# pierluigiferrari/fcn8s_tensorflow

Hardware: AMD Instinct MI355X
Metric: training images/sec at 1024x512 bs16 (higher is better)
Workload: dtype f32; 1 GPU; FCN-8s (VGG-16, fc6 7x7, 20 classes) train step, 1024x512, 16 images/GPU, SGD+momentum, keep_prob 0.5; global_batch=16, parallelism=dp1

## Files before the change

fcn8s_tensorflow_amd/csrc/elementwise.hip:

```cpp
#include "fcn8s_internal.h"
#include "cv_resize.h"
#include <math.h>
#include <map>
#include <mutex>
#include <stdio.h>
#include <stdlib.h>

namespace fcn8s {

static inline int cap_blocks(long long work, int per_block)
{
    long long b = (work + per_block - 1) / per_block;
    if (b > 2048) b = 2048;
    if (b < 1) b = 1;
    return (int)b;
}

__global__ void preprocess_kernel(const void* img, int dtype, float4* out, long long npix)
{
    const float m0 = 103.939f, m1 = 116.779f, m2 = 123.68f;
    for (long long p = blockIdx.x * (long long)blockDim.x + threadIdx.x; p < npix;
         p += (long long)gridDim.x * blockDim.x) {
        float r, g, b;
        if (dtype == 0) {
// ... 419 lines not shown
            const float4* src = reinterpret_cast<const float4*>(logits) + p0 * U;
#pragma unroll
            for (int i = 0; i < U; ++i) { const int u = i * 64 + lane; if (p0 * U + u < nunits) wp[u] = src[u]; }
            __builtin_amdgcn_wave_barrier();
#pragma unroll
            for (int i = 0; i < U; ++i) { const float4 t = wp[lane * U + i]; v[4*i] = t.x; v[4*i+1] = t.y; v[4*i+2] = t.z; v[4*i+3] = t.w; }
            __builtin_amdgcn_wave_barrier();
        } else {
            const float4 t = p < npix ? reinterpret_cast<const float4*>(logits)[p] : make_float4(0.f, 0.f, 0.f, 0.f);
            v[0] = t.x; v[1] = t.y; v[2] = t.z; v[3] = t.w;
        }
        float4 g[U];
#pragma unroll
        for (int i = 0; i < U; ++i) g[i] = make_float4(0.f, 0.f, 0.f, 0.f);
        if (pix >= 0) {
            float m = v[0];
#pragma unroll
            for (int i = 1; i < C; ++i) m = fmaxf(m, v[i]);
            float e[C]; float s = 0.f;
#pragma unroll
            for (int i = 0; i < C; ++i) { e[i] = expf(v[i] - m); s += e[i]; }
            const int lab = labels[pix];
            const bool ign = lab >= C;
            float vl = 0.f;
#pragma unroll
            for (int i = 0; i < C; ++i) vl = (i == lab) ? v[i] : vl;
            float gs = gscale;
            bool keep = !ign;
            if constexpr (PH == XENT_PLAIN) {
                if (!ign) lsum += (double)(m + logf(s) - vl);
            } else if constexpr (PH == XENT_WEIGHTED) {
                float w = ign ? 0.f : wsh[lab];
                if constexpr (PX) w *= tab[x.codes[pix]];
                gs = gscale * w; nv += !ign;
                if (!ign) lsum += (double)w * (double)(m + logf(s) - vl);
            } else if constexpr (PH == XENT_OHEM_LOSS) {
                const float l = m + logf(s) - vl;
                if (!ign) { ++nv; ntau += l >= x.tau; atomicAdd(&hsh[__float_as_uint(l) >> 21], 1u); }
                x.lbuf[pix] = ign ? -1.f : l;
            } else {
                const float l = x.lbuf[pix];
                keep = !ign && l >= tsel;
                float w = keep ? wsh[lab] : 0.f;
                if constexpr (PX) w *= tab[x.codes[pix]];
                gs = gsel * w;
                if (keep) lsum += (double)w * (double)l;
            }
            if (PH != XENT_OHEM_LOSS && dlogits) {
                const float inv = keep ? gs / s : 0.f;
#pragma unroll
                for (int i = 0; i < U; ++i) {
                    float4 t;
                    t.x = e[4*i] * inv - ((4*i) == lab ? gs : 0.f);
                    t.y = e[4*i+1] * inv - ((4*i+1) == lab ? gs : 0.f);
                    t.z = e[4*i+2] * inv - ((4*i+2) == lab ? gs : 0.f);
                    t.w = e[4*i+3] * inv - ((4*i+3) == lab ? gs : 0.f);
                    g[i] = t;
                    csum[4*i] += t.x; csum[4*i+1] += t.y; csum[4*i+2] += t.z; csum[4*i+3] += t.w;
                }
            }
        }
        if (PH != XENT_OHEM_LOSS && dlogits) {
            if constexpr (U > 1) {
#pragma unroll
                for (int i = 0; i < U; ++i) wp[lane * U + i] = g[i];
                __builtin_amdgcn_wave_barrier();
                float4* dst = reinterpret_cast<float4*>(dlogits) + p0 * U;
#pragma unroll
                for (int i = 0; i < U; ++i) { const int u = i * 64 + lane; if (p0 * U + u < nunits) dst[u] = wp[u]; }
                __builtin_amdgcn_wave_barrier();
            } else if (p < npix) reinterpret_cast<float4*>(dlogits)[p] = g[0];
        }
    }
    if constexpr (PH == XENT_WEIGHTED || PH == XENT_OHEM_LOSS) xent_fold<PH>(nv, ntau, cnt, hsh, x);
// ... 697 lines not shown
```

fcn8s_tensorflow_amd/csrc/fcn8s_internal.h:

```cpp
#pragma once
#include <hip/hip_runtime.h>
#include <stdint.h>
#include <cmath>
#include "../../include/fcn8s_hip.h"

#if defined(__HIP_DEVICE_COMPILE__) && !defined(__gfx950__)
#error "libfcn8s_hip is written for gfx950 (MI355X) only: build with --offload-arch=gfx950"
#endif
#define FCN8S_LDS_BYTES_NEEDED (160u * 1024u)

#include <string>
namespace fcn8s {

extern thread_local const char* g_last_kernel;
void defer_error(int code, const char* fmt, ...) __attribute__((format(printf, 2, 3)));
int take_deferred_error(std::string* text);

struct IgemmArgs {
    const float* x; const float* w; const float* bias; const float* addend; const float* mask;
    float* y;
    int N, Ma, Mb; long long M;
    int Hi, Wi, Cin, ldx;
    int KW, in_scale, tap_step, tap_off, Ktot;
    int Ho, Wo, Cout, ldy;
// ... 147 lines not shown
void launch_lovasz_backward(const float* x, int is_logits, const uint8_t* labels, const PixMap* map, int N, long long npix, const LovaszLayout& y,
                            char* ws, float lambda, int accumulate, float* out, float* colsum, hipStream_t s);
void launch_lovasz_total(float* terms, float lce, float* loss_out, hipStream_t s);
size_t soft_targets_scratch_bytes();
double soft_targets_bytes(long long npix, int C, int K);
void launch_soft_targets(const float* logits, float* dlogits, const float* probs, const uint8_t* labels, const PixMap* map, int N, long long npix, int C,
                         int K, long long row_stride, float lambda, float temperature, int all_pixels, char* ws, float* loss, float* term,
                         float* lastbias, hipStream_t s);
void launch_softmax_argmax(const float* logits, float* softmax_out, long long* argmax_out,
                           long long npix, int C, hipStream_t s, const PixMap* map = nullptr, int N = 0);
void launch_tconv_im2col(const float* x, float* A, int N, int Hi, int Wi, int C, int KP, hipStream_t s);
void launch_tconv_col2im(const float* dA, float* dx, int N, int Hi, int Wi, int C, int KP, hipStream_t s);
void launch_tconv_pack_gemm(const float* w, const float* bias, float* b2, float* b2t, float* bias_tiled, int C, int S, int KP, hipStream_t s);
void launch_tconv_unpack_dw(const float* db2, float* dw, int C, int S, hipStream_t s);
void launch_unblock_logits(const float* blocked, float* nhwc, const PixMap& map, int N, int C, hipStream_t s);
void launch_onehot_to_ids(const void* oh, int elem_bytes, long long npix, int C, uint8_t* ids, int* bad, hipStream_t s);
void launch_confusion(const uint8_t* labels, const long long* pred, long long npix,
                      unsigned long long* conf, int C, hipStream_t s);
bool launch_head_fwd(const float* x, const float* w, const float* bias, float* y, long long M, int K, int C, float alpha, hipStream_t s,
                     float* scratch = nullptr, size_t scratch_floats = 0);
bool launch_head_dgrad(const float* dy, const float* wt, const float* mask, float mask_scale, float* dx, long long M, int K, int C, float alpha,
                       hipStream_t s);
bool launch_head_wgrad(const float* x, const float* dy, float* dw, long long M, int K, int C, float alpha, hipStream_t s);
bool launch_maxpool_bwd_bf16(const float* x, const float* dy, unsigned short* dzb, float* db, int N, int H, int W, int C, hipStream_t s, const unsigned char* route = nullptr, long long dzb_ps = 0);
void launch_colsum(const float* x, float* out, long long rows, int C, hipStream_t s);
void launch_sumsq(const float* x, float* out, long long n, hipStream_t s);
void launch_axpy(float* y, const float* x, float a, long long n, hipStream_t s);
void launch_grad_accumulate(float* dst, const float* src, long long n, int mode, hipStream_t s);
constexpr int kGradNormBlocks = 2048;
struct UpdateStats { float norm, clip, scale; int ok; unsigned long long skipped; };
// ... 106 lines not shown
```

fcn8s_tensorflow_amd/csrc/model.hip:

```cpp
#include "../../include/fcn8s_hip.h"
#include "fcn8s_internal.h"
#include "device_buffer.h"
#include "pass_state.h"
#include "conv_route.h"
#include <cstdarg>
#include <functional>

#include <dlfcn.h>
#include <atomic>
#include <chrono>
#include <thread>
#include <cmath>
#include <cstdio>
#include <cstring>
#include <cstdlib>
#include <algorithm>
#include <mutex>
#include <map>
#include <set>
#include <string>
#include <vector>

using namespace fcn8s;

// ... 139 lines not shown
    bool mc_masks = false;
    hipStream_t stream = nullptr;
    std::set<hipStream_t> streams_seen; hipEvent_t move_ev = nullptr;
    int64_t step = 0;
    int N = 0, H = 0, W = 0;
    int plan_N = 0;
    DeviceBuf<char> arena;
    std::map<std::string, Act> acts;
    std::vector<Layer> layers;
    struct KeptDy { DeviceBuf<float> p; size_t n = 0; };
    int keep_dy = 0; std::map<std::string, KeptDy> kept_dy;
    int tconv_gemm = 1; PixMap pm{0, 0, 0, 0, 0, 0}; int tg_kp = 0;
    float *logits_b = nullptr, *dlogits_b = nullptr, *tg_A = nullptr, *tg_dA = nullptr;
    DeviceBuf<float> tg_b2, tg_b2t, tg_bias, tg_db2;
    bool logits_nhwc_valid = false;
    float *dlogits = nullptr, *da3 = nullptr, *da4 = nullptr, *ds7 = nullptr, *gskip3 = nullptr, *gskip4 = nullptr;
    float *gbuf[2] = {nullptr, nullptr};
    int gcur = 0;
    void* d_images = nullptr; uint8_t* d_labels = nullptr;
    DeviceBuf<float> d_loss; float *d_regsum = nullptr, *d_softmax = nullptr;
    PinnedBuf<float> h_loss; hipEvent_t loss_ev = nullptr; bool loss_copied = false;
    float* d_lastbias = nullptr;
    double* d_partials = nullptr; long long* d_pred = nullptr;
    int loss_mode = 0, last_loss_mode = 0; float ohem_thresh = 0.f; int64_t ohem_min_kept = 0;
    DeviceBuf<float> d_cw; DeviceBuf<char> loss_ws;
    int bnd_R = 0; long long bnd_last = 0; DeviceBuf<float> d_btab; DeviceBuf<uint8_t> d_bcodes;
    bool lov_on = false, have_terms = false; float lov_ce = 1.f, lov_w = 0.f; int lov_per_image = 0, lov_all = 0;
    DeviceBuf<uint8_t> d_lovmask; int lov_nmask = 0; DeviceBuf<char> lov_ws; float* d_terms = nullptr;
    float kd_w = 0.f, kd_T = 1.f; int kd_all = 0; bool have_kd = false;
    const float* kd_probs = nullptr; int kd_N = 0, kd_H = 0, kd_W = 0, kd_K = 0; long long kd_stride = 0;
// ... 850 lines not shown

    size_t bytes = 0;
    for (auto& it : items) { pl.offs.push_back(bytes); bytes = align_up(bytes + it.n * sizeof(float), 256); }
    const size_t npix = (size_t)N * H * W;
    pl.o_img = bytes;  bytes = align_up(bytes + npix * 3 * sizeof(float), 256);
    pl.o_lab = bytes;  bytes = align_up(bytes + npix, 256);
    pl.o_pred = bytes; bytes = align_up(bytes + npix * sizeof(long long), 256);
    pl.o_part = bytes; bytes = align_up(bytes + 4096 * sizeof(double), 256);
    pl.bytes = bytes;
}
void carve_workspace(fcn8s_model* m, int N, int H, int W, const WsPlan& pl)
{
    m->acts.clear();
    m->have_forward = m->have_loss = false;
    m->pm = PixMap{m->tconv_gemm ? 1 : 0, H, W, H / 8 + 1, W / 8 + 1, 8};
    m->logits_b = m->dlogits_b = m->tg_A = m->tg_dA = nullptr;
    m->d_wino_v = m->d_wino_m = nullptr;
    for (size_t i = 0; i < pl.items.size(); ++i) {
        float* p = (float*)(m->arena + pl.offs[i]);
        if (pl.items[i].extra) *pl.items[i].extra = p;
        Act a; a.p = p; a.n = pl.items[i].n; a.H = pl.items[i].h; a.W = pl.items[i].w; a.C = pl.items[i].c;
        m->acts[pl.items[i].name] = a;
    }
    m->layers = pl.layers;
    auto view = [&](int i) { return i < 0 ? nullptr : (float*)(m->arena + pl.offs[i]); };
    for (Layer& L : m->layers) { L.y = view(L.i_y); L.wv = view(L.i_wv); L.pool = view(L.i_pool); L.rb = (unsigned*)view(L.i_rb); L.pidx = (unsigned char*)view(L.i_pidx); }
    m->d_images = m->arena + pl.o_img; m->d_labels = (uint8_t*)(m->arena + pl.o_lab);
    m->d_pred = (long long*)(m->arena + pl.o_pred); m->d_partials = (double*)(m->arena + pl.o_part);
    m->N = N; m->H = H; m->W = W;
}
void drop_arena(fcn8s_model* m)
{
    if (m->arena) hipStreamSynchronize(m->stream);
    m->arena.reset();
    m->N = m->H = m->W = 0; m->acts.clear();
    for (Layer& L : m->layers) { L.y = L.wv = L.pool = nullptr; L.rb = nullptr; L.pidx = nullptr; }
    m->have_forward = m->have_loss = false;
}
void drop_shape_copies(fcn8s_model* m, bool keep_regrowable = false)
{
    if (!m->xbf16.empty() || (!keep_regrowable && !(m->xg16.empty() && m->dyg16.empty() && m->q8.empty()))) hipStreamSynchronize(m->stream);
    m->xbf16.clear();
    m->pass.forget_shape_copies(keep_regrowable);
    if (keep_regrowable) {
        for (auto& kv : m->xg16) m->g16_stale.insert("x:" + kv.first);
        for (auto& kv : m->dyg16) m->g16_stale.insert("d:" + kv.first);
        return;
    }
    m->xg16.clear(); m->dyg16.clear(); m->g16_stale.clear();
    m->q8.clear();
}
void drop_banks(fcn8s_model* m, bool keep_w8 = false)
// ... 35 lines not shown
    if (same && m->arena.bytes() >= bytes) return FCN8S_OK;
    WsPlan pl;
    plan_workspace(m, N, H, W, pl);
    bytes = std::max(bytes, pl.bytes);
    if (m->arena.bytes() < bytes) {
        drop_arena(m);
        if (!m->arena.grow(bytes, m->stream, &m->ws_allocs)) return fail(m, FCN8S_ERR_OOM, "workspace hipMalloc failed: out of memory");
    }
    if (!same) drop_shape_copies(m, true);
    carve_workspace(m, N, H, W, pl);
    return FCN8S_OK;
}

float* A(fcn8s_model* m, const char* n) { return m->acts.at(n).p; }

const float* LG(fcn8s_model* m) { return (m->tconv_gemm && m->logits_b) ? m->logits_b : m->acts.at("logits").p; }
const PixMap* LGM(fcn8s_model* m) { return (m->tconv_gemm && m->logits_b) ? &m->pm : nullptr; }
IgemmArgs tg_rows_gemm(const float* x, int ldx, int K, const float* w, float* y, int ncols, long long rows)
{
    IgemmArgs a{};
    a.x = x; a.w = w; a.y = y;
    a.N = 1; a.Ma = (int)rows; a.Mb = 1; a.M = rows;
    a.Hi = (int)rows; a.Wi = 1; a.Cin = K; a.ldx = ldx;
    a.KW = 1; a.in_scale = 1; a.tap_step = 1; a.tap_off = 0; a.Ktot = K;
    a.Ho = (int)rows; a.Wo = 1; a.Cout = ncols; a.ldy = ncols;
    a.out_scale = 1; a.phases_x = 1; a.alpha = 1.f; a.mask_scale = 1.f;
    return a;
}
void tconv_gemm_fwd(fcn8s_model* m)
{
    hipStream_t s = m->stream;
    const int C = m->C, NC = 64 * C, KP = m->tg_kp;
    const long long rows = (long long)m->N * m->pm.QH * m->pm.QW;
    ProfScope ps(m, "tconv_fwd", 2.0 * rows * 4 * C * NC, 4.0 * rows * (4.0 * C + NC));
    launch_tconv_pack_gemm(Wp(m, "fc7_pool4_pool3_conv2d_trans/kernel"), Wp(m, "fc7_pool4_pool3_conv2d_trans/bias"), m->tg_b2, m->tg_b2t, m->tg_bias, C, 8, KP, s);
    launch_tconv_im2col(m->acts.at("a3").p, m->tg_A, m->N, m->H / 8, m->W / 8, C, KP, s);
    IgemmArgs a = tg_rows_gemm(m->tg_A, KP, 4 * C, m->tg_b2, m->logits_b, NC, rows);
    a.split = split_of(m);
    a.bias = m->tg_bias;
    launch_igemm(a, 1, s);
}
void tconv_gemm_dgrad(fcn8s_model* m)
{
    hipStream_t s = m->stream;
    const int C = m->C, NC = 64 * C, KP = m->tg_kp;
    const long long rows = (long long)m->N * m->pm.QH * m->pm.QW;
    ProfScope ps(m, "tconv_dgrad", 2.0 * rows * NC * KP, 4.0 * rows * (NC + KP));
    IgemmArgs a = tg_rows_gemm(m->dlogits_b, NC, NC, m->tg_b2t, m->tg_dA, KP, rows);
    a.split = split_of(m);
    a.batched = 1;
    launch_igemm(a, 1, s);
    launch_tconv_col2im(m->tg_dA, m->da3, m->N, m->H / 8, m->W / 8, C, KP, s);
}
void tconv_gemm_wgrad(fcn8s_model* m)
{
// ... 446 lines not shown
        if (xb7 && !fuse7) { ProfScope ps(m, "bf16_convert", 0, 6.0 * N * h5 * w5 * F7.cin); launch_f32_to_bf16_padded(F6.y, xb7, N, h5, w5, F7.cin, 0, s, g16_ps(N, h5, w5, 1)); }
        if (!bf16_conv_layer(m, "fc7_fwd_bf16", F7, F6.y, F7.y, s, io7)) return fwd_failed(fail(m, FCN8S_ERR_SHAPE, "bf16_train: fc7 does not fit the bf16 convolution kernel"));
    } else if (m->precision == FCN8S_PREC_BF16_FC || bf16_fwd_mode(m)) {
        bf16_conv_layer(m, "fc6_fwd_bf16", F6, x, F6.y, s, io6);
        if (train) wino_backward_operands(m, F6.name, x, w6, N, h5, w5, F6.cin, F6.cout, F6.K, s);
        bf16_conv_layer(m, "fc7_fwd_bf16", F7, F6.y, F7.y, s, io7);
    } else {
        { FwdEpi e; e.bias = b6; e.relu = 1; e.dropout = drop; e.keep = keep_prob; e.stream_id = m->drop_stream;
          conv_fwd(m, "fc6_fwd", x, w6, F6.y, N, h5, w5, F6.cin, F6.cout, F6.K, e, s, 0, F6.name); }
        { FwdEpi e; e.bias = b7; e.relu = 1; e.dropout = drop; e.keep = keep_prob; e.stream_id = m->drop_stream + 1;
          conv_fwd(m, "fc7_fwd", F6.y, w7, F7.y, N, h5, w5, F7.cin, F7.cout, 1, e, s); }
    }
    return FwdStep{};
}

struct FwdCall { float keep_prob = 1.f; bool train = false, x0_written = false, calibrating = false; const McLoop* mc = nullptr; };

int forward(fcn8s_model* m, const void* img_dev, int dtype, const FwdCall& call)
{
    const float keep_prob = call.keep_prob; const bool train = call.train; const McLoop* mc = call.mc;
    t_deterministic = m->deterministic;
    hipStream_t s = m->stream;
    const int N = m->N, H = m->H, W = m->W, C = m->C;
    const bool fp8 = fp8_mode(m) && !train && !call.calibrating;
    if (fp8 && !m->fp8_calibrated)
        return fail(m, FCN8S_ERR_STATE, "fp8_infer: the model has no FP8 calibration (never calibrated, or its parameters changed since): run fcn8s_fp8_calibrate "
                                        "(Engine.calibrate_fp8 / FCN8s.calibrate_fp8) or restore one with fcn8s_fp8_set_calibration first");
    m->pass.begin_forward(fp8);
    bool guard_pending = false;
    if (m->frozen && keeps_banks(m) && !m->banks_stale) {
        launch_fingerprint(m->d_params, (long long)m->total, m->d_fp, s);
// ... 36 lines not shown
        if (st.rc) return st.rc;
        x = last.pool;
    }
    const int h5 = H / 32, w5 = W / 32;
    auto skip_heads = [&]() {
        { FwdEpi e; e.bias = Wp(m, "pool3_1x1/bias"); e.alpha = 0.0001f;
          conv_fwd(m, "score1x1_fwd", A(m, "pool3"), Wp(m, "pool3_1x1/kernel"), A(m, "p3"), N, H / 8, W / 8, m->widths[2], C, 1, e, s); }
        { FwdEpi e; e.bias = Wp(m, "pool4_1x1/bias"); e.alpha = 0.01f;
          conv_fwd(m, "score1x1_fwd", A(m, "pool4"), Wp(m, "pool4_1x1/kernel"), A(m, "p4"), N, H / 16, W / 16, m->widths[3], C, 1, e, s); }
    };
    auto fc7_head_and_upsampling = [&]() {
        { FwdEpi e; e.bias = Wp(m, "fc7_1x1/bias");
          conv_fwd(m, "score1x1_fwd", A(m, "fc7"), Wp(m, "fc7_1x1/kernel"), A(m, "s7"), N, h5, w5, m->widths[6], C, 1, e, s); }
        tconv_fwd(m, A(m, "s7"), m->d_tph[0], Wp(m, "fc7_conv2d_trans/bias"), A(m, "p4"), A(m, "a4"), N, h5, w5, C, 4, 2, s);
        tconv_fwd(m, A(m, "a4"), m->d_tph[1], Wp(m, "fc7_pool4_conv2d_trans/bias"), A(m, "p3"), A(m, "a3"), N, H / 16, W / 16, C, 4, 2, s);
        if (m->tconv_gemm && m->logits_b) tconv_gemm_fwd(m);
        else tconv_fwd(m, A(m, "a3"), m->d_tph[2], Wp(m, "fc7_pool4_pool3_conv2d_trans/bias"), nullptr, A(m, "logits"), N, H / 8, W / 8, C, 16, 8, s);
        m->logits_nhwc_valid = !(m->tconv_gemm && m->logits_b);
    };
    if (!mc) {
        { const FwdStep st = fwd_fc(m, x, keep_prob, train, fp8, bo); if (st.rc) return st.rc; }
        skip_heads();
        fc7_head_and_upsampling();
    } else {
        skip_heads();
        for (int k = 0; k < mc->samples; ++k) {
            const uint32_t sid = mc->stream_base + 2u * (uint32_t)k;
            const FwdStep st = fwd_fc(m, x, keep_prob, train, fp8, bo, &sid); if (st.rc) return st.rc;
            fc7_head_and_upsampling();
            mc->after_sample(k);
        }
// ... 95 lines not shown
    return m->loss_ws.grow(need, m->stream, &m->ws_allocs) ? FCN8S_OK : fail(m, FCN8S_ERR_OOM, "the training loss's scratch cannot be allocated");
}

int ensure_lovasz_ws(fcn8s_model* m, const LovaszLayout& y)
{
    return m->lov_ws.grow(y.bytes, m->stream, &m->ws_allocs) ? FCN8S_OK : fail(m, FCN8S_ERR_OOM, "the Lovasz sort's scratch cannot be allocated");
}

int compute_loss(fcn8s_model* m, const uint8_t* lab_dev, float l2_rate, bool with_grad)
{
    hipStream_t s = m->stream;
    const long long npix = (long long)m->N * m->H * m->W;
    const int nb = softmax_xent_blocks(npix);
    const bool bnd = with_grad && m->bnd_R > 0;
    const int mode = with_grad ? (m->loss_mode ? m->loss_mode : bnd ? 1 : 0) : 0;
    if (mode) { int rc = ensure_loss_ws(m, npix, mode); if (rc) return rc; }
    if (bnd) {
        if ((long long)m->H * m->W >= (1LL << 31)) return fail(m, FCN8S_ERR_SHAPE, "fcn8s_set_boundary_loss: an image has to have fewer than 2^31 pixels");
        if (!m->d_btab || !m->d_cw) return fail(m, FCN8S_ERR_STATE, "fcn8s_set_boundary_loss: the table is missing");
        if (!m->d_bcodes.grow((size_t)npix, s, &m->ws_allocs)) return fail(m, FCN8S_ERR_OOM, "the boundary weighting's distance codes cannot be allocated");
        ProfScope ps(m, "boundary_distance", 0, 2.0 * (double)npix);
        launch_boundary_distance(lab_dev, m->N, m->H, m->W, m->bnd_R, m->d_bcodes, s);
    }
    OhemState* st = mode ? (OhemState*)m->loss_ws.get() : nullptr;
    const bool lov = with_grad && m->lov_on;
    const bool lov_sort = lov && m->lov_w != 0.f;
    const float gscale = lov ? m->lov_ce * (1.0f / (float)npix) : 1.0f / (float)npix;
    LovaszLayout ly;
    if (lov_sort) {
        if (npix / (m->lov_per_image ? m->N : 1) >= (1LL << 31)) return fail(m, FCN8S_ERR_BAD_ARG, "fcn8s_set_lovasz: a segment holds 2^31 pixels or more");
        ly = lovasz_layout(npix, m->lov_per_image ? m->N : 1, m->C);
        int rc = ensure_lovasz_ws(m, ly); if (rc) return rc;
    }
    const double xbytes = (mode == 2 ? (double)npix * (m->C * 4 * 3 + 2 + 8) : (double)npix * (m->C * 4 * (with_grad ? 2 : 1) + 1)) + (bnd ? (double)npix : 0.0);
    { ProfScope ps(m, "softmax_xent", 0, xbytes);
      if (with_grad) hipMemsetAsync(m->d_lastbias, 0, 64 * sizeof(float), s);
      const bool blk = m->tconv_gemm && m->logits_b;
      if (mode) {
          XentEx x; x.cw = m->d_cw; x.st = st; x.hist = (unsigned*)(m->loss_ws + sizeof(OhemState));
          x.lbuf = mode == 2 ? (float*)(m->loss_ws + LOSS_SCRATCH_BYTES) : nullptr;
          if (lov) x.ce_scale = m->lov_ce;
          if (bnd) { x.codes = m->d_bcodes; x.ptab = m->d_btab; }
          launch_softmax_xent_ex(blk ? m->logits_b : A(m, "logits"), lab_dev, blk ? m->dlogits_b : m->dlogits, m->d_partials, npix, m->C, gscale, s,
                                 m->d_lastbias, blk ? &m->pm : nullptr, m->N, x, mode == 2 ? m->ohem_thresh : 0.f, (long long)m->ohem_min_kept);
      } else
          launch_softmax_xent(blk ? m->logits_b : A(m, "logits"), lab_dev, with_grad ? (blk ? m->dlogits_b : m->dlogits) : nullptr, m->d_partials, npix, m->C,
                              gscale, s, with_grad ? m->d_lastbias : nullptr, blk ? &m->pm : nullptr, m->N); }
    if (with_grad) { m->last_loss_mode = mode; m->bnd_last = bnd ? npix : 0; }
    const float* reg = nullptr;
// ... 387 lines not shown
    for (int i = 0; i < n; ++i)
        if (!std::isfinite(amax[i]) || amax[i] < 0.f) return fail(m, FCN8S_ERR_BAD_ARG, "fcn8s_fp8_set_calibration: maxima must be finite and >= 0");
    memcpy(m->fp8_amax, amax, sizeof m->fp8_amax);
    m->fp8_calibrated = true;
    return FCN8S_OK;
}

static int* model_option(fcn8s_model* m, const std::string& key)
{
    if (key == "winograd_min_cin") return &m->wino_min_cin;
    if (key == "winograd_tile") return &m->wino_tile;
    if (key == "winograd_fc6") return &m->wino_fc6;
    if (key == "fc6_fft") return &m->fc6_fft;
    if (key == "fc6_fft_wgrad") return &m->fc6_fft_wgrad;
    if (key == "tconv_gemm") return &m->tconv_gemm;
    if (key == "fuse_dgrad_dout") return &m->fuse_dgrad_dout;
    if (key == "fuse_out_in") return &m->fuse_out_in;
    if (key == "bf16_gemm256") return &m->bf16_gemm256;
    if (key == "winograd_tile_hires") return &m->wino_tile_hires;
    if (key == "winograd_hires_pixels") return &m->wino_hires_pixels;
    if (key == "conv1_tiled") return &m->conv1_tiled;
    if (key == "conv1_wgrad_mfma") return &m->conv1_wgrad_mfma;
    if (key == "bf16_copy_by_transform") return &m->bf16_copy_by_transform;
    if (key == "conv1_in_transform") return &m->conv1_in_transform;
    if (key == "deterministic") return &m->deterministic;
    if (key == "bf16_acts") return &m->bf16_acts;
    if (key == "bf16_rows_bn") return &m->bf16_rows_bn;
    if (key == "keep_output_gradients") return &m->keep_dy;
    if (key == "bf16_infer_copies") return &m->bf16_infer_copies;
    if (key == "bf16_fuse_pool") return &m->bf16_fuse_pool;
// ... 8 lines not shown
        if (k == "op_f32x3") { t_op_split = value ? 3 : 0; return FCN8S_OK; }
        if (k == "op_deterministic") { t_deterministic = value ? 1 : 0; return FCN8S_OK; }
        if (k == "op_bf16_planes") { t_op_planes = value ? 1 : 0; return FCN8S_OK; }
        if (k == "op_bf16_rows_bn") { if (value != 0 && value != 64 && value != 128) return fail(nullptr, FCN8S_ERR_BAD_ARG, "op_bf16_rows_bn must be 0, 64 or 128"); t_op_rows_bn = (int)value; return FCN8S_OK; }
        if (k == "op_split_pieces") {
            if (value != 0 && value != 2 && value != 3) return fail(nullptr, FCN8S_ERR_BAD_ARG, "fcn8s_set_option: op_split_pieces is 0, 2 or 3");
            t_op_split = (int)value; return FCN8S_OK;
        }
        return fail(nullptr, FCN8S_ERR_NOT_FOUND, "fcn8s_set_option: unknown op-context option '" + k + "' (model options need a model)");
    }
    if (k == "workspace_allocations" || k == "frozen") return fail(m, FCN8S_ERR_BAD_ARG, "fcn8s_set_option: '" + k + "' is read-only (the frozen state is set with fcn8s_freeze_params)");
    if (k == "comm_timeout_ms") {
        if (value < 1) return fail(m, FCN8S_ERR_BAD_ARG, "comm_timeout_ms must be >= 1");
        std::lock_guard<std::mutex> lk(m->comm_mu); m->comm_timeout_ms = value; return FCN8S_OK;
    }
    if (k == "conv1_tiled" || k == "conv1_wgrad_mfma" || k == "bf16_copy_by_transform" || k == "conv1_in_transform" || k == "deterministic" || k == "bf16_acts" || k == "bf16_rows_bn" || k == "bf16_fuse_pool" || k == "keep_output_gradients" || k == "bf16_infer_copies") {
        *model_option(m, k) = k == "bf16_rows_bn" ? (int)value : (value ? 1 : 0);
        return FCN8S_OK;
    }
    int* slot = model_option(m, k);
    if (!slot) return fail(m, FCN8S_ERR_NOT_FOUND, "fcn8s_set_option: unknown option '" + k + "'");
    if (direct_mode(m->precision) && (k == "winograd_min_cin" || k == "winograd_fc6")) {
        if (value < 0) return fail(m, FCN8S_ERR_BAD_ARG, "fcn8s_set_option: negative value");
        (k == "winograd_min_cin" ? m->saved_wino_min_cin : m->saved_wino_fc6) = (int)value;
        return FCN8S_OK;
    }
    if (k == "winograd_tile" && value != 2 && value != 4 && value != 6) return fail(m, FCN8S_ERR_BAD_ARG, "winograd_tile must be 2, 4 or 6");
    if (k == "winograd_tile_hires" && value != 0 && value != 2 && value != 4 && value != 6) return fail(m, FCN8S_ERR_BAD_ARG, "winograd_tile_hires must be 0, 2, 4 or 6");
    if (k == "winograd_min_cin" && value < 0) return fail(m, FCN8S_ERR_BAD_ARG, "winograd_min_cin must be >= 0 (0 = direct convolution everywhere)");
    if (k == "fuse_out_in" && (value < 0 || value > 2)) return fail(m, FCN8S_ERR_BAD_ARG, "fuse_out_in must be 0, 1 or 2");
    if (k == "fc6_fft_wgrad" && (value < 0 || value > 2)) return fail(m, FCN8S_ERR_BAD_ARG, "fc6_fft_wgrad must be 0, 1 or 2");
// ... 125 lines not shown

int fcn8s_forward_loss(fcn8s_model* m, const void* images, int dtype, const uint8_t* labels, int N, int H, int W,
                       float keep_prob, float l2_rate, int where)
{
    if (fp8_mode(m)) return fp8_refuse_training(m, "fcn8s_forward_loss");
    if (m && m->frozen) fcn8s_freeze_params(m, 0);
    fp8_clear_calibration(m);
    if (!m || !images || !labels) return fail(m, FCN8S_ERR_BAD_ARG, "fcn8s_forward_loss: null argument");
    if (!(keep_prob > 0.f && keep_prob <= 1.f)) return fail(m, FCN8S_ERR_BAD_ARG, "keep_prob must be in (0, 1]");
    if (m->kd_w != 0.f) {
        if (!m->kd_probs) return fail(m, FCN8S_ERR_STATE, "fcn8s_set_soft_targets is on and no targets are bound: call fcn8s_bind_soft_targets before every training loss");
        if (m->kd_N != N || m->kd_H != H || m->kd_W != W)
            return fail(m, FCN8S_ERR_SHAPE, "the bound soft targets are for a batch of " + std::to_string(m->kd_N) + " x " + std::to_string(m->kd_H) + " x " +
                        std::to_string(m->kd_W) + ", the training loss for " + std::to_string(N) + " x " + std::to_string(H) + " x " + std::to_string(W));
    }
    FwdCall call; call.keep_prob = keep_prob; call.train = true;
    const uint8_t* lab;
    int rc = run_pass(m, images, dtype, labels, N, H, W, where, call, &lab); if (rc) return rc;
    rc = compute_loss(m, lab, l2_rate, true); if (rc) return rc;
    m->kd_probs = nullptr;
    m->next_bucket = 0;
    for (int b = 0; b < kNumBuckets; ++b) m->acc_taken[b] = false;
    HIPCHK(m, hipGetLastError());
    return FCN8S_OK;
}

int fcn8s_backward_bucket(fcn8s_model* m, int bucket)
{
    if (!m || bucket < 0 || bucket >= kNumBuckets) return fail(m, FCN8S_ERR_BAD_ARG, "bad bucket");
    if (fp8_mode(m)) return fp8_refuse_training(m, "fcn8s_backward_bucket");
    take_deferred_error(nullptr);
// ... 1008 lines not shown
            const double v = (e == 15 && mt == 7) ? NAN : (e ? ldexp(1.0 + mt / 8.0, e - 7) : ldexp((double)mt, -9));
            lut[c] = (float)ldexp((c & 128) ? -v : v, b.ex);
        }
        const int Hp = b.H + 2 * b.pad, Wq = b.W + 2 * b.pad;
        for (int nn = 0; nn < b.N; ++nn)
            for (int y = 0; y < b.H; ++y)
                for (int x = 0; x < b.W; ++x) {
                    const long long q = ((long long)nn * Hp + y + b.pad) * Wq + x + b.pad;
                    float* dst = host + (((size_t)nn * b.H + y) * b.W + x) * b.C;
                    for (int c = 0; c < b.C; ++c) dst[c] = lut[raw[(size_t)(c >> 6) * b.ps + q * 64 + (c & 63)]];
                }
        return FCN8S_OK;
    }
    auto it = m->acts.find(name);
    if (it == m->acts.end()) return fail(m, FCN8S_ERR_NOT_FOUND, std::string("unknown activation '") + name + "'");
    if (std::string(name) == "logits" && !m->logits_nhwc_valid && m->logits_b) {
        launch_unblock_logits(m->logits_b, it->second.p, m->pm, m->N, m->C, m->stream);
        m->logits_nhwc_valid = true;
    }
    if (n != it->second.n) return fail(m, FCN8S_ERR_SHAPE, std::string("activation '") + name + "' has " + std::to_string(it->second.n) + " elements");
    if (m->pass.y_unwritten.count(name))
        return fail(m, FCN8S_ERR_STATE, std::string("activation '") + name + "' was not materialised by the last forward pass: " +
                                        (fp8_mode(m) ? std::string("fp8_infer keeps it only as its consumer's e4m3 copy (fcn8s_get_activation(m, \"q8:<consumer>\", ...))") :
                                         bf16_train_mode(m) ? "bf16_train keeps a conv -> conv activation only as the consumer's padded bf16 copy (option \"bf16_acts\" = 0 keeps the fp32 tensor too)" :
                                         std::string(name) == "conv1_1" ? "conv1_2's input transform evaluated it on its own patches (option \"conv1_in_transform\" = 0 keeps it)"
                                                                        : "its output transform wrote the next conv's transformed input directly (option \"fuse_out_in\" = 0 keeps it)"));
    HIPCHK(m, hipStreamSynchronize(m->stream));
    HIPCHK(m, hipMemcpy(host, it->second.p, n * sizeof(float), hipMemcpyDeviceToHost));
    return FCN8S_OK;
}
// ... 707 lines not shown
```

Measured before the change: 294.7 images/sec.

## Fuse final transposed-conv GEMM with softmax cross-entropy loss and gradient

Adds a kernel that computes the final 16x transposed convolution as an MFMA GEMM tile and immediately applies per-pixel softmax cross-entropy, writing only dlogits and loss partials. Training forward passes defer the logits GEMM, and the loss stage runs the fused kernel when the configuration allows it (C=20, blocked pixel map, plain loss). This avoids writing the full-resolution logits tensor and reading it back in a separate loss pass. Logits are still produced on demand if something asks for them. The per-pixel softmax math moves into a shared header.

```diff
diff --git a/fcn8s_tensorflow_amd/csrc/elementwise.hip b/fcn8s_tensorflow_amd/csrc/elementwise.hip
--- a/fcn8s_tensorflow_amd/csrc/elementwise.hip
+++ b/fcn8s_tensorflow_amd/csrc/elementwise.hip
@@ -1,5 +1,6 @@
 #include "fcn8s_internal.h"
 #include "cv_resize.h"
+#include "xent_pixel.h"
 #include <math.h>
 #include <map>
 #include <mutex>
@@ -457,28 +458,21 @@
 #pragma unroll
         for (int i = 0; i < U; ++i) g[i] = make_float4(0.f, 0.f, 0.f, 0.f);
         if (pix >= 0) {
-            float m = v[0];
-#pragma unroll
-            for (int i = 1; i < C; ++i) m = fmaxf(m, v[i]);
-            float e[C]; float s = 0.f;
-#pragma unroll
-            for (int i = 0; i < C; ++i) { e[i] = expf(v[i] - m); s += e[i]; }
             const int lab = labels[pix];
             const bool ign = lab >= C;
-            float vl = 0.f;
-#pragma unroll
-            for (int i = 0; i < C; ++i) vl = (i == lab) ? v[i] : vl;
+            float m, s, vl, e[C];
+            xent_softmax<C>(v, lab, m, e, s, vl);
             float gs = gscale;
             bool keep = !ign;
             if constexpr (PH == XENT_PLAIN) {
-                if (!ign) lsum += (double)(m + logf(s) - vl);
+                if (!ign) lsum += (double)xent_pixel_loss(m, s, vl);
             } else if constexpr (PH == XENT_WEIGHTED) {
                 float w = ign ? 0.f : wsh[lab];
                 if constexpr (PX) w *= tab[x.codes[pix]];
                 gs = gscale * w; nv += !ign;
-                if (!ign) lsum += (double)w * (double)(m + logf(s) - vl);
+                if (!ign) lsum += (double)w * (double)xent_pixel_loss(m, s, vl);
             } else if constexpr (PH == XENT_OHEM_LOSS) {
-                const float l = m + logf(s) - vl;
+                const float l = xent_pixel_loss(m, s, vl);
                 if (!ign) { ++nv; ntau += l >= x.tau; atomicAdd(&hsh[__float_as_uint(l) >> 21], 1u); }
                 x.lbuf[pix] = ign ? -1.f : l;
             } else {
@@ -491,16 +485,7 @@
             }
             if (PH != XENT_OHEM_LOSS && dlogits) {
                 const float inv = keep ? gs / s : 0.f;
-#pragma unroll
-                for (int i = 0; i < U; ++i) {
-                    float4 t;
-                    t.x = e[4*i] * inv - ((4*i) == lab ? gs : 0.f);
-                    t.y = e[4*i+1] * inv - ((4*i+1) == lab ? gs : 0.f);
-                    t.z = e[4*i+2] * inv - ((4*i+2) == lab ? gs : 0.f);
-                    t.w = e[4*i+3] * inv - ((4*i+3) == lab ? gs : 0.f);
-                    g[i] = t;
-                    csum[4*i] += t.x; csum[4*i+1] += t.y; csum[4*i+2] += t.z; csum[4*i+3] += t.w;
-                }
+                xent_grad<C>(e, inv, gs, lab, g, csum);
             }
         }
         if (PH != XENT_OHEM_LOSS && dlogits) {
diff --git a/fcn8s_tensorflow_amd/csrc/fcn8s_internal.h b/fcn8s_tensorflow_amd/csrc/fcn8s_internal.h
--- a/fcn8s_tensorflow_amd/csrc/fcn8s_internal.h
+++ b/fcn8s_tensorflow_amd/csrc/fcn8s_internal.h
@@ -185,6 +185,9 @@
 void launch_tconv_pack_gemm(const float* w, const float* bias, float* b2, float* b2t, float* bias_tiled, int C, int S, int KP, hipStream_t s);
 void launch_tconv_unpack_dw(const float* db2, float* dw, int C, int S, hipStream_t s);
 void launch_unblock_logits(const float* blocked, float* nhwc, const PixMap& map, int N, int C, hipStream_t s);
+bool tconv_xent_covers(int C, const PixMap& map, int N);
+void launch_tconv_softmax_xent(const float* A, int lda, const float* b2, const float* bias_tiled, const uint8_t* labels, float* dlogits,
+                               double* partials, long long npix, int N, const PixMap& map, float grad_scale, float* colsum, hipStream_t s);
 void launch_onehot_to_ids(const void* oh, int elem_bytes, long long npix, int C, uint8_t* ids, int* bad, hipStream_t s);
 void launch_confusion(const uint8_t* labels, const long long* pred, long long npix,
                       unsigned long long* conf, int C, hipStream_t s);
diff --git a/fcn8s_tensorflow_amd/csrc/model.hip b/fcn8s_tensorflow_amd/csrc/model.hip
--- a/fcn8s_tensorflow_amd/csrc/model.hip
+++ b/fcn8s_tensorflow_amd/csrc/model.hip
@@ -177,6 +177,7 @@
     float *logits_b = nullptr, *dlogits_b = nullptr, *tg_A = nullptr, *tg_dA = nullptr;
     DeviceBuf<float> tg_b2, tg_b2t, tg_bias, tg_db2;
     bool logits_nhwc_valid = false;
+    int tconv_fuse_loss = 1; bool logits_deferred = false;
     float *dlogits = nullptr, *da3 = nullptr, *da4 = nullptr, *ds7 = nullptr, *gskip3 = nullptr, *gskip4 = nullptr;
     float *gbuf[2] = {nullptr, nullptr};
     int gcur = 0;
@@ -1057,7 +1058,7 @@
     m->acts.clear();
     m->have_forward = m->have_loss = false;
     m->pm = PixMap{m->tconv_gemm ? 1 : 0, H, W, H / 8 + 1, W / 8 + 1, 8};
-    m->logits_b = m->dlogits_b = m->tg_A = m->tg_dA = nullptr;
+    m->logits_b = m->dlogits_b = m->tg_A = m->tg_dA = nullptr; m->logits_deferred = false;
     m->d_wino_v = m->d_wino_m = nullptr;
     for (size_t i = 0; i < pl.items.size(); ++i) {
         float* p = (float*)(m->arena + pl.offs[i]);
@@ -1078,7 +1079,7 @@
     m->arena.reset();
     m->N = m->H = m->W = 0; m->acts.clear();
     for (Layer& L : m->layers) { L.y = L.wv = L.pool = nullptr; L.rb = nullptr; L.pidx = nullptr; }
-    m->have_forward = m->have_loss = false;
+    m->have_forward = m->have_loss = false; m->logits_deferred = false;
 }
 void drop_shape_copies(fcn8s_model* m, bool keep_regrowable = false)
 {
@@ -1144,7 +1145,8 @@
 
 float* A(fcn8s_model* m, const char* n) { return m->acts.at(n).p; }
 
-const float* LG(fcn8s_model* m) { return (m->tconv_gemm && m->logits_b) ? m->logits_b : m->acts.at("logits").p; }
+void ensure_logits(fcn8s_model* m);
+const float* LG(fcn8s_model* m) { ensure_logits(m); return (m->tconv_gemm && m->logits_b) ? m->logits_b : m->acts.at("logits").p; }
 const PixMap* LGM(fcn8s_model* m) { return (m->tconv_gemm && m->logits_b) ? &m->pm : nullptr; }
 IgemmArgs tg_rows_gemm(const float* x, int ldx, int K, const float* w, float* y, int ncols, long long rows)
 {
@@ -1157,18 +1159,39 @@
     a.out_scale = 1; a.phases_x = 1; a.alpha = 1.f; a.mask_scale = 1.f;
     return a;
 }
-void tconv_gemm_fwd(fcn8s_model* m)
+bool fuse_loss_route(const fcn8s_model* m)
+{
+    return m->tconv_fuse_loss && m->tconv_gemm && m->logits_b && split_of(m) == 0 && tconv_xent_covers(m->C, m->pm, m->N) &&
+           !m->loss_mode && m->bnd_R <= 0 && !m->lov_on && m->kd_w == 0.f;
+}
+static void tconv_gemm_logits(fcn8s_model* m)
+{
+    const int C = m->C, NC = 64 * C, KP = m->tg_kp;
+    const long long rows = (long long)m->N * m->pm.QH * m->pm.QW;
+    IgemmArgs a = tg_rows_gemm(m->tg_A, KP, 4 * C, m->tg_b2, m->logits_b, NC, rows);
+    a.split = split_of(m);
+    a.bias = m->tg_bias;
+    launch_igemm(a, 1, m->stream);
+}
+void tconv_gemm_fwd(fcn8s_model* m, bool defer)
 {
     hipStream_t s = m->stream;
     const int C = m->C, NC = 64 * C, KP = m->tg_kp;
     const long long rows = (long long)m->N * m->pm.QH * m->pm.QW;
-    ProfScope ps(m, "tconv_fwd", 2.0 * rows * 4 * C * NC, 4.0 * rows * (4.0 * C + NC));
+    ProfScope ps(m, "tconv_fwd", defer ? 0.0 : 2.0 * rows * 4 * C * NC, defer ? 4.0 * rows * (C + 4.0 * C) : 4.0 * rows * (4.0 * C + NC));
     launch_tconv_pack_gemm(Wp(m, "fc7_pool4_pool3_conv2d_trans/kernel"), Wp(m, "fc7_pool4_pool3_conv2d_trans/bias"), m->tg_b2, m->tg_b2t, m->tg_bias, C, 8, KP, s);
     launch_tconv_im2col(m->acts.at("a3").p, m->tg_A, m->N, m->H / 8, m->W / 8, C, KP, s);
-    IgemmArgs a = tg_rows_gemm(m->tg_A, KP, 4 * C, m->tg_b2, m->logits_b, NC, rows);
-    a.split = split_of(m);
-    a.bias = m->tg_bias;
-    launch_igemm(a, 1, s);
+    if (!defer) tconv_gemm_logits(m);
+    m->logits_deferred = defer;
+}
+void ensure_logits(fcn8s_model* m)
+{
+    if (!m->logits_deferred || !m->logits_b) return;
+    t_deterministic = m->deterministic;
+    const long long rows = (long long)m->N * m->pm.QH * m->pm.QW;
+    ProfScope ps(m, "tconv_fwd", 2.0 * rows * 4 * m->C * 64 * m->C, 4.0 * rows * (4.0 * m->C + 64 * m->C));
+    tconv_gemm_logits(m);
+    m->logits_deferred = false;
 }
 void tconv_gemm_dgrad(fcn8s_model* m)
 {
@@ -1645,7 +1668,8 @@
     return FwdStep{};
 }
 
-struct FwdCall { float keep_prob = 1.f; bool train = false, x0_written = false, calibrating = false; const McLoop* mc = nullptr; };
+struct FwdCall { float keep_prob = 1.f; bool train = false, x0_written = false, calibrating = false; const McLoop* mc = nullptr;
+                 bool fused_loss = false; };
 
 int forward(fcn8s_model* m, const void* img_dev, int dtype, const FwdCall& call)
 {
@@ -1712,7 +1736,7 @@
           conv_fwd(m, "score1x1_fwd", A(m, "fc7"), Wp(m, "fc7_1x1/kernel"), A(m, "s7"), N, h5, w5, m->widths[6], C, 1, e, s); }
         tconv_fwd(m, A(m, "s7"), m->d_tph[0], Wp(m, "fc7_conv2d_trans/bias"), A(m, "p4"), A(m, "a4"), N, h5, w5, C, 4, 2, s);
         tconv_fwd(m, A(m, "a4"), m->d_tph[1], Wp(m, "fc7_pool4_conv2d_trans/bias"), A(m, "p3"), A(m, "a3"), N, H / 16, W / 16, C, 4, 2, s);
-        if (m->tconv_gemm && m->logits_b) tconv_gemm_fwd(m);
+        if (m->tconv_gemm && m->logits_b) tconv_gemm_fwd(m, call.fused_loss && fuse_loss_route(m));
         else tconv_fwd(m, A(m, "a3"), m->d_tph[2], Wp(m, "fc7_pool4_pool3_conv2d_trans/bias"), nullptr, A(m, "logits"), N, H / 8, W / 8, C, 16, 8, s);
         m->logits_nhwc_valid = !(m->tconv_gemm && m->logits_b);
     };
@@ -1838,6 +1862,8 @@
     const int nb = softmax_xent_blocks(npix);
     const bool bnd = with_grad && m->bnd_R > 0;
     const int mode = with_grad ? (m->loss_mode ? m->loss_mode : bnd ? 1 : 0) : 0;
+    const bool fused = with_grad && m->logits_deferred && fuse_loss_route(m);
+    if (!fused) ensure_logits(m);
     if (mode) { int rc = ensure_loss_ws(m, npix, mode); if (rc) return rc; }
     if (bnd) {
         if ((long long)m->H * m->W >= (1LL << 31)) return fail(m, FCN8S_ERR_SHAPE, "fcn8s_set_boundary_loss: an image has to have fewer than 2^31 pixels");
@@ -1857,6 +1883,14 @@
         int rc = ensure_lovasz_ws(m, ly); if (rc) return rc;
     }
     const double xbytes = (mode == 2 ? (double)npix * (m->C * 4 * 3 + 2 + 8) : (double)npix * (m->C * 4 * (with_grad ? 2 : 1) + 1)) + (bnd ? (double)npix : 0.0);
+    if (fused) {
+        const double rows = (double)m->N * m->pm.QH * m->pm.QW;
+        ProfScope ps(m, "tconv_fwd_xent", 2.0 * rows * 4 * m->C * 64 * m->C, 4.0 * rows * (4.0 * m->C + 64 * m->C) + (double)npix);
+        hipMemsetAsync(m->d_lastbias, 0, 64 * sizeof(float), s);
+        launch_tconv_softmax_xent(m->tg_A, m->tg_kp, m->tg_b2, m->tg_bias, lab_dev, m->dlogits_b, m->d_partials, npix, m->N, m->pm, gscale,
+                                  m->deterministic ? nullptr : m->d_lastbias, s);
+        if (m->deterministic) launch_colsum(m->dlogits_b, m->d_lastbias, pixmap_slots(m->pm, npix, m->N), m->C, s);
+    } else
     { ProfScope ps(m, "softmax_xent", 0, xbytes);
       if (with_grad) hipMemsetAsync(m->d_lastbias, 0, 64 * sizeof(float), s);
       const bool blk = m->tconv_gemm && m->logits_b;
@@ -2274,6 +2308,7 @@
     if (key == "fc6_fft") return &m->fc6_fft;
     if (key == "fc6_fft_wgrad") return &m->fc6_fft_wgrad;
     if (key == "tconv_gemm") return &m->tconv_gemm;
+    if (key == "tconv_fuse_loss") return &m->tconv_fuse_loss;
     if (key == "fuse_dgrad_dout") return &m->fuse_dgrad_dout;
     if (key == "fuse_out_in") return &m->fuse_out_in;
     if (key == "bf16_gemm256") return &m->bf16_gemm256;
@@ -2312,7 +2347,7 @@
         if (value < 1) return fail(m, FCN8S_ERR_BAD_ARG, "comm_timeout_ms must be >= 1");
         std::lock_guard<std::mutex> lk(m->comm_mu); m->comm_timeout_ms = value; return FCN8S_OK;
     }
-    if (k == "conv1_tiled" || k == "conv1_wgrad_mfma" || k == "bf16_copy_by_transform" || k == "conv1_in_transform" || k == "deterministic" || k == "bf16_acts" || k == "bf16_rows_bn" || k == "bf16_fuse_pool" || k == "keep_output_gradients" || k == "bf16_infer_copies") {
+    if (k == "conv1_tiled" || k == "conv1_wgrad_mfma" || k == "bf16_copy_by_transform" || k == "conv1_in_transform" || k == "deterministic" || k == "bf16_acts" || k == "bf16_rows_bn" || k == "bf16_fuse_pool" || k == "keep_output_gradients" || k == "bf16_infer_copies" || k == "tconv_fuse_loss") {
         *model_option(m, k) = k == "bf16_rows_bn" ? (int)value : (value ? 1 : 0);
         return FCN8S_OK;
     }
@@ -2468,7 +2503,7 @@
             return fail(m, FCN8S_ERR_SHAPE, "the bound soft targets are for a batch of " + std::to_string(m->kd_N) + " x " + std::to_string(m->kd_H) + " x " +
                         std::to_string(m->kd_W) + ", the training loss for " + std::to_string(N) + " x " + std::to_string(H) + " x " + std::to_string(W));
     }
-    FwdCall call; call.keep_prob = keep_prob; call.train = true;
+    FwdCall call; call.keep_prob = keep_prob; call.train = true; call.fused_loss = true;
     const uint8_t* lab;
     int rc = run_pass(m, images, dtype, labels, N, H, W, where, call, &lab); if (rc) return rc;
     rc = compute_loss(m, lab, l2_rate, true); if (rc) return rc;
@@ -3507,6 +3542,7 @@
     }
     auto it = m->acts.find(name);
     if (it == m->acts.end()) return fail(m, FCN8S_ERR_NOT_FOUND, std::string("unknown activation '") + name + "'");
+    if (std::string(name) == "logits") ensure_logits(m);
     if (std::string(name) == "logits" && !m->logits_nhwc_valid && m->logits_b) {
         launch_unblock_logits(m->logits_b, it->second.p, m->pm, m->N, m->C, m->stream);
         m->logits_nhwc_valid = true;
diff --git a/fcn8s_tensorflow_amd/csrc/tconv_xent.hip b/fcn8s_tensorflow_amd/csrc/tconv_xent.hip
--- /dev/null
+++ b/fcn8s_tensorflow_amd/csrc/tconv_xent.hip
@@ -0,0 +1,176 @@
+#include "fcn8s_internal.h"
+#include "xent_pixel.h"
+
+namespace fcn8s {
+
+typedef float tx_f32x16 __attribute__((ext_vector_type(16)));
+
+struct TconvXentArgs {
+    const float* A; int lda;
+    const float* B;
+    const float* bias;
+    const uint8_t* labels;
+    float* dlogits;
+    double* partials;
+    float* colsum;
+    long long rows; int ntiles;
+    int H, W, QH, QW;
+    float gscale;
+};
+
+constexpr int TX_C = 20, TX_K = 4 * TX_C, TX_NC = 64 * TX_C, TX_BM = 128, TX_BN = 8 * TX_C, TX_TN = TX_BN / 32, TX_NCH = TX_NC / TX_BN;
+
+__global__ __launch_bounds__(256, 2) void tconv_softmax_xent_kernel(const TconvXentArgs p)
+{
+    constexpr int C = TX_C, U = C / 4, BN = TX_BN, TN = TX_TN, NB4 = TX_K * BN / 4, BLD = (NB4 + 255) / 256;
+    __shared__ __attribute__((aligned(16))) float sB[TX_K * BN];
+    __shared__ __attribute__((aligned(16))) float sP[4 * 8 * BN];
+    __shared__ double sh[4];
+    __shared__ float cs[C];
+    const int tid = threadIdx.x, lane = tid & 63, wave = __builtin_amdgcn_readfirstlane(tid >> 6);
+    const int half = lane >> 5, l31 = lane & 31;
+    float csum[C];
+#pragma unroll
+    for (int i = 0; i < C; ++i) csum[i] = 0.f;
+    if (tid < C) cs[tid] = 0.f;
+    double lsum = 0;
+    float* patch = sP + wave * 8 * BN;
+
+    float4 af[TX_K / 8];
+#define TX_LOAD_A(t_)                                                                                                             \
+    {                                                                                                                             \
+        long long mr = (long long)((t_) / TX_NCH) * TX_BM + wave * 32 + l31; if (mr >= p.rows) mr = p.rows - 1;                   \
+        const float4* ap = reinterpret_cast<const float4*>(p.A + mr * p.lda) + half;                                              \
+        _Pragma("unroll") for (int i = 0; i < TX_K / 8; ++i) af[i] = ap[2 * i];                                                   \
+    }
+    int cur_ch = -1;
+    float bv[TN];
+    if ((int)blockIdx.x < p.ntiles) TX_LOAD_A((int)blockIdx.x)
+    for (int t = blockIdx.x; t < p.ntiles; t += gridDim.x) {
+        const int ch = t % TX_NCH;
+        const long long m0 = (long long)(t / TX_NCH) * TX_BM;
+        if (ch != cur_ch) {
+            float4 tb[BLD];
+#pragma unroll
+            for (int i = 0; i < BLD; ++i) {
+                const int u = i * 256 + tid, k = u / (BN / 4), c4 = u - k * (BN / 4);
+                if (u < NB4) tb[i] = *reinterpret_cast<const float4*>(p.B + (long long)k * TX_NC + ch * BN + c4 * 4);
+            }
+            if (cur_ch >= 0) __syncthreads();
+#pragma unroll
+            for (int i = 0; i < BLD; ++i) { const int u = i * 256 + tid; if (u < NB4) reinterpret_cast<float4*>(sB)[u] = tb[i]; }
+#pragma unroll
+            for (int tn = 0; tn < TN; ++tn) bv[tn] = p.bias[ch * BN + tn * 32 + l31];
+            cur_ch = ch;
+            __syncthreads();
+        }
+
+        int labs[4];
+#pragma unroll
+        for (int g8 = 0; g8 < 4; ++g8) {
+            const long long mm = m0 + wave * 32 + g8 * 8 + (lane >> 3);
+            labs[g8] = -1;
+            if (mm < p.rows) {
+                const unsigned mu = (unsigned)mm, tq = mu / (unsigned)p.QW;
+                const int qx = (int)(mu - tq * (unsigned)p.QW);
+                const long long n = tq / (unsigned)p.QH;
+                const int q = (int)(tq - (unsigned)n * (unsigned)p.QH);
+                const int oy = q * 8 - 4 + ch, ox = qx * 8 - 4 + (lane & 7);
+                if ((unsigned)oy < (unsigned)p.H && (unsigned)ox < (unsigned)p.W) labs[g8] = p.labels[(n * p.H + oy) * p.W + ox];
+            }
+        }
+        tx_f32x16 acc[TN];
+#pragma unroll
+        for (int tn = 0; tn < TN; ++tn)
+#pragma unroll
+            for (int r = 0; r < 16; ++r) acc[tn][r] = 0.f;
+#pragma unroll
+        for (int i = 0; i < TX_K / 8; ++i) {
+            float bf[TN][4];
+#pragma unroll
+            for (int tn = 0; tn < TN; ++tn)
+#pragma unroll
+                for (int j = 0; j < 4; ++j) bf[tn][j] = sB[(i * 8 + half * 4 + j) * BN + tn * 32 + l31];
+#pragma unroll
+            for (int j = 0; j < 4; ++j) {
+                const float av = j == 0 ? af[i].x : j == 1 ? af[i].y : j == 2 ? af[i].z : af[i].w;
+#pragma unroll
+                for (int tn = 0; tn < TN; ++tn) acc[tn] = __builtin_amdgcn_mfma_f32_32x32x2f32(av, bf[tn][j], acc[tn], 0, 0, 0);
+            }
+        }
+
+#pragma unroll
+        for (int g8 = 0; g8 < 4; ++g8) {
+            if (g8 == 2 && t + (int)gridDim.x < p.ntiles) TX_LOAD_A(t + (int)gridDim.x)
+#pragma unroll
+            for (int tn = 0; tn < TN; ++tn)
+#pragma unroll
+                for (int r4 = 0; r4 < 4; ++r4) patch[(r4 + 4 * half) * BN + tn * 32 + l31] = acc[tn][g8 * 4 + r4] + bv[tn];
+            __builtin_amdgcn_wave_barrier();
+            const long long mrow = m0 + wave * 32 + g8 * 8;
+            {
+                const int rl = lane >> 3, px = lane & 7;
+                float4* pv = reinterpret_cast<float4*>(patch + rl * BN + px * C);
+                float4 g[U];
+#pragma unroll
+                for (int i = 0; i < U; ++i) g[i] = make_float4(0.f, 0.f, 0.f, 0.f);
+                const int lab = labs[g8];
+                if (lab >= 0) {
+                    float v[C];
+#pragma unroll
+                    for (int i = 0; i < U; ++i) { const float4 w = pv[i]; v[4*i] = w.x; v[4*i+1] = w.y; v[4*i+2] = w.z; v[4*i+3] = w.w; }
+                    const bool ign = lab >= C;
+                    float m, s, vl, e[C];
+                    xent_softmax<C>(v, lab, m, e, s, vl);
+                    if (!ign) lsum += (double)xent_pixel_loss(m, s, vl);
+                    const float gs = p.gscale;
+                    const float inv = !ign ? gs / s : 0.f;
+                    xent_grad<C>(e, inv, gs, lab, g, csum);
+                }
+#pragma unroll
+                for (int i = 0; i < U; ++i) pv[i] = g[i];
+            }
+            __builtin_amdgcn_wave_barrier();
+            float* dst = p.dlogits + ch * BN;
+#pragma unroll
+            for (int i = 0; i < 8 * BN / 4 / 64; ++i) {
+                const int u = i * 64 + lane, rl = u / (BN / 4), c4 = u - rl * (BN / 4);
+                const float4 w = *reinterpret_cast<const float4*>(patch + rl * BN + c4 * 4);
+                if (mrow + rl < p.rows) *reinterpret_cast<float4*>(dst + (mrow + rl) * TX_NC + c4 * 4) = w;
+            }
+            __builtin_amdgcn_wave_barrier();
+        }
+    }
+
+#undef TX_LOAD_A
+    for (int o = 32; o > 0; o >>= 1) lsum += __shfl_down(lsum, o, 64);
+    if (lane == 0) sh[wave] = lsum;
+    __syncthreads();
+    if (tid == 0) p.partials[blockIdx.x] = sh[0] + sh[1] + sh[2] + sh[3];
+    if (p.colsum) {
+#pragma unroll
+        for (int i = 0; i < C; ++i) {
+            float v = csum[i];
+#pragma unroll
+            for (int o = 32; o > 0; o >>= 1) v += __shfl_down(v, o, 64);
+            if (lane == 0) atomicAdd(&cs[i], v);
+        }
+        __syncthreads();
+        if (tid < C) unsafeAtomicAdd(p.colsum + tid, cs[tid]);
+    }
+}
+
+bool tconv_xent_covers(int C, const PixMap& pm, int N) { return C == TX_C && pm.blocked && pm.S == 8 && (long long)N * pm.QH * pm.QW < (1LL << 31); }
+
+void launch_tconv_softmax_xent(const float* A, int lda, const float* b2, const float* bias_tiled, const uint8_t* labels, float* dlogits,
+                               double* partials, long long npix, int N, const PixMap& pm, float grad_scale, float* colsum, hipStream_t s)
+{
+    TconvXentArgs a{};
+    a.A = A; a.lda = lda; a.B = b2; a.bias = bias_tiled; a.labels = labels; a.dlogits = dlogits; a.partials = partials; a.colsum = colsum;
+    a.rows = (long long)N * pm.QH * pm.QW;
+    a.ntiles = (int)((a.rows + TX_BM - 1) / TX_BM) * TX_NCH;
+    a.H = pm.H; a.W = pm.W; a.QH = pm.QH; a.QW = pm.QW;
+    a.gscale = grad_scale;
+    hipLaunchKernelGGL(tconv_softmax_xent_kernel, dim3(softmax_xent_blocks(npix)), dim3(256), 0, s, a);
+}
+}
diff --git a/fcn8s_tensorflow_amd/csrc/xent_pixel.h b/fcn8s_tensorflow_amd/csrc/xent_pixel.h
--- /dev/null
+++ b/fcn8s_tensorflow_amd/csrc/xent_pixel.h
@@ -0,0 +1,31 @@
+#pragma once
+#include <hip/hip_runtime.h>
+
+template <int C>
+static __device__ __forceinline__ void xent_softmax(const float (&v)[C], int lab, float& m, float (&e)[C], float& s, float& vl)
+{
+    m = v[0];
+#pragma unroll
+    for (int i = 1; i < C; ++i) m = fmaxf(m, v[i]);
+    s = 0.f;
+#pragma unroll
+    for (int i = 0; i < C; ++i) { e[i] = expf(v[i] - m); s += e[i]; }
+    vl = 0.f;
+#pragma unroll
+    for (int i = 0; i < C; ++i) vl = (i == lab) ? v[i] : vl;
+}
+static __device__ __forceinline__ float xent_pixel_loss(float m, float s, float vl) { return m + logf(s) - vl; }
+template <int C>
+static __device__ __forceinline__ void xent_grad(const float (&e)[C], float inv, float gs, int lab, float4 (&g)[C / 4], float (&csum)[C])
+{
+#pragma unroll
+    for (int i = 0; i < C / 4; ++i) {
+        float4 t;
+        t.x = e[4*i] * inv - ((4*i) == lab ? gs : 0.f);
+        t.y = e[4*i+1] * inv - ((4*i+1) == lab ? gs : 0.f);
+        t.z = e[4*i+2] * inv - ((4*i+2) == lab ? gs : 0.f);
+        t.w = e[4*i+3] * inv - ((4*i+3) == lab ? gs : 0.f);
+        g[i] = t;
+        csum[4*i] += t.x; csum[4*i+1] += t.y; csum[4*i+2] += t.z; csum[4*i+3] += t.w;
+    }
+}
```

New measurement: 295.1 images/sec, median of 2. Within noise of the previous version (+0.1%).
